# jhidalgocarrio/slam-localization

Hardware: AMD Instinct MI355X
Metric: filter predict+update steps/sec (higher is better)
Workload: dtype f64

## Files before the change

### slam-localization_amd/csrc/slk_kernels.hpp

```cpp
#pragma once
#include <hip/hip_runtime.h>

#include "../../include/slk.h"
#include "slk_math.hpp"

namespace slk {

typedef double d4 __attribute__((ext_vector_type(4)));
typedef float f4 __attribute__((ext_vector_type(4)));
typedef __bf16 b8 __attribute__((ext_vector_type(8)));

constexpr int KP = 8;
constexpr int STEP_WGS = 4;
constexpr int MAXM = 32;
constexpr int PRED_SCRATCH = 1536;

struct Lay { int kind, k, nfk, nfkl, N, Nq, nso3; };

struct KArgs {
    int B;
    Lay lay;
    double *mean; double *P; int *status; unsigned *outliers;
    int do_predict, pm; const double *u; int u_stride; const double *Q; int q_stride; const double *Yext;
    int do_update, mm; const double *mp; int mp_stride; const double *z; int m;
// ... 478 lines not shown
                        if (rho < kap) f = 0.0;
                        frag[I] = f;
                        if (rho >= kap && rho < n && kap < n) Lp[pk(n, rho, kap)] = f;
                    }
#pragma unroll
                    for (int J = JK; J < NT; ++J)
#pragma unroll
                        for (int I = J; I < NT; ++I)
                            acc[tile_idx(I, J)] = __builtin_amdgcn_mfma_f64_16x16x4f64(frag[I], frag[J], acc[tile_idx(I, J)], 0, 0, 0);
                }
            }
            CholMCols<NT, JK + 1>::run(acc, Lp, n, colbuf, lane, fail);
        }
    }
};

template <int NT>
__device__ __forceinline__ int cholm_factor(d4 (&acc)[CholM<NT>::NTL], double *Lp, int n, double *colbuf, int lane)
{
    int fail = -1;
    __builtin_amdgcn_s_setprio(3);
    CholMCols<NT, 0>::run(acc, Lp, n, colbuf, lane, fail);
    wave_sync();
    __builtin_amdgcn_s_setprio(0);
    return fail;
}

__device__ __forceinline__ double readlane_f64(double x, int l)
{
    return __hiloint2double(__builtin_amdgcn_readlane(__double2hiint(x), l), __builtin_amdgcn_readlane(__double2loint(x), l));
}

template <int J> __device__ __forceinline__ double row_bcast_const_f64(double x)
{
    return __builtin_amdgcn_update_dpp(0.0, x, 0x150 + J, 0xf, 0xf, true);
}
__device__ __forceinline__ double row_bcast_f64(double x, int j)
{
    switch (j & 15) {
    case 0: return row_bcast_const_f64<0>(x);
    case 1: return row_bcast_const_f64<1>(x);
    case 2: return row_bcast_const_f64<2>(x);
    case 3: return row_bcast_const_f64<3>(x);
    case 4: return row_bcast_const_f64<4>(x);
    case 5: return row_bcast_const_f64<5>(x);
    case 6: return row_bcast_const_f64<6>(x);
    case 7: return row_bcast_const_f64<7>(x);
    case 8: return row_bcast_const_f64<8>(x);
    case 9: return row_bcast_const_f64<9>(x);
    case 10: return row_bcast_const_f64<10>(x);
    case 11: return row_bcast_const_f64<11>(x);
    case 12: return row_bcast_const_f64<12>(x);
    case 13: return row_bcast_const_f64<13>(x);
    case 14: return row_bcast_const_f64<14>(x);
    default: return row_bcast_const_f64<15>(x);
    }
}

template <int LO, int HI, int OFF>
__device__ __forceinline__ void lds_store4_lane_ranges(unsigned addr, const double (&v)[4])
{
    constexpr int W0 = HI - LO > 0 ? HI - LO : 0, W1 = HI - LO - 1 > 0 ? HI - LO - 1 : 0;
    constexpr int W2 = HI - LO - 2 > 0 ? HI - LO - 2 : 0, W3 = HI - LO - 3 > 0 ? HI - LO - 3 : 0;
    static_assert(LO >= 0 && HI <= 64 && W0 < 64 && LO + 3 < 64 && OFF >= 0 && OFF + 384 < 65536, "s_bfm_b64 fields, ds offset");
    unsigned long long save;
    asm volatile("s_mov_b64 %[sv], exec\n\t"
                 "s_bfm_b64 exec, %[w0], %[l0]\n\tds_write_b64 %[a], %[v0] offset:%[o0]\n\t"
                 "s_bfm_b64 exec, %[w1], %[l1]\n\tds_write_b64 %[a], %[v1] offset:%[o1]\n\t"
                 "s_bfm_b64 exec, %[w2], %[l2]\n\tds_write_b64 %[a], %[v2] offset:%[o2]\n\t"
                 "s_bfm_b64 exec, %[w3], %[l3]\n\tds_write_b64 %[a], %[v3] offset:%[o3]\n\t"
                 "s_mov_b64 exec, %[sv]"
                 : [sv] "=&s"(save)
                 : [a] "v"(addr), [v0] "v"(v[0]), [v1] "v"(v[1]), [v2] "v"(v[2]), [v3] "v"(v[3]),
                   [w0] "n"(W0), [w1] "n"(W1), [w2] "n"(W2), [w3] "n"(W3), [l0] "n"(LO), [l1] "n"(LO + 1), [l2] "n"(LO + 2), [l3] "n"(LO + 3),
                   [o0] "n"(OFF), [o1] "n"(OFF + 128), [o2] "n"(OFF + 256), [o3] "n"(OFF + 384)
                 : "memory");
}

struct CholNoRelease { __device__ __forceinline__ void operator()() const { } };
template <int NT, int JK, int C0, int OUT = 1, int NC = 0>
struct CholPSteps {
    template <class RelFn>
    __device__ __forceinline__ static void run(d4 (&acc)[CholM<NT>::NTL], double *Lp, int n, double *colbuf, int lane, unsigned &bad,
                                               int ksync, RelFn &rel)
    {
        static_assert(OUT != 2 || (NC > 0 && NC <= 16 * NT), "the tile variant takes n as a template argument too");
        if constexpr (JK < NT) {
            constexpr int LDC = CholM<NT>::LDC;
            constexpr int k0 = 16 * JK + C0;
            if constexpr (OUT == 2) n = NC;
            if (k0 < n) {
                const int c = lane & 15, g = lane >> 4;
                const int row = (NT == 4) ? lane : min(lane, 16 * NT - 1);
                auto live = [&](int p) { return OUT != 2 || k0 + p < n; };
                const bool last = OUT == 2 && k0 + 4 >= n;
#pragma unroll
                for (int I = JK; I < NT; ++I) colbuf[g * LDC + 16 * I + c] = acc[tile_idx(I, JK)][C0 / 4];
                wave_sync();
                double m[4], l[4];
#pragma unroll
                for (int p = 0; p < 4; ++p) m[p] = live(p) ? colbuf[p * LDC + row] : 0.0;
#pragma unroll
                for (int p = 0; p < 4; ++p) {
                    l[p] = 0.0;
                    if (!live(p)) continue;
                    const double mpiv = readlane_f64(m[p], k0 + p), d = -mpiv;
                    {
                        if constexpr (OUT == 2) {
                            const unsigned rk = pivot_rank_neg((unsigned)__double2hiint(mpiv), (unsigned)__double2loint(mpiv));
                            bad = rk > bad ? rk : bad;
                            asm volatile("" : "+s"(bad));
                        } else {
                            int nb = !(d > 0.0);
                            asm volatile("" : "+v"(nb));
                            bad |= (nb != 0) ? 0x7ff00000u : 0u;
                        }
                    }
                    double sq, rs;
                    rsqrt_pivot(d, sq, rs);
                    (void)sq;
                    l[p] = m[p] * -rs;
#pragma unroll
                    for (int q = p + 1; q < 4; ++q)
                        if (live(q)) m[q] = fma(l[p], readlane_f64(l[p], k0 + q), m[q]);
                }
                if constexpr (OUT != 2) {
                    wave_sync();
                    if (NT == 4 || lane < 16 * NT) {
#pragma unroll
                        for (int p = 0; p < 4; ++p) colbuf[p * LDC + lane] = l[p];
                    }
                }
                if constexpr (OUT == 2) {
                    typedef __attribute__((address_space(3))) double ldouble;
                    const int It = lane >> 4;
                    const unsigned trow = (unsigned)(size_t)(ldouble *)Lp + (It * (It + 1) / 2 * 256 + (lane & 15)) * 8;
                    lds_store4_lane_ranges<k0, NC, (JK * 256 + C0 * 16) * 8>(trow, l);
                    if (ksync == k0 / 4) rel();
                }
#pragma unroll
                for (int p = 0; p < 4; ++p) {
                    if constexpr (OUT == 1) {
                        typedef __attribute__((address_space(1))) double gdouble;
                        unsigned long long colb = reinterpret_cast<unsigned long long>(Lp + pkcol(n, k0 + p));
                        asm volatile("" : "+s"(colb));
                        gdouble *colp = reinterpret_cast<gdouble *>(colb);
                        if (k0 + p < n && lane >= k0 + p && lane < n) colp[lane] = l[p];
                    } else if constexpr (OUT == 0) {
                        if (k0 + p < n && lane >= k0 + p && lane < n) Lp[pkcol(n, k0 + p) + lane] = l[p];
                    }
                }
                if (!last) {
                    constexpr int J0 = (C0 == 12) ? JK + 1 : JK;
                    wave_sync();
                    double frag[NT];
                    if constexpr (OUT == 2) {
#pragma unroll
                        for (int I = J0; I < NT; ++I) frag[I] = Lp[tile_idx(I, JK) * 256 + (C0 + g) * 16 + c];
                    } else {
#pragma unroll
                        for (int I = J0; I < NT; ++I) frag[I] = colbuf[g * LDC + 16 * I + c];
                        wave_sync();
                    }
#pragma unroll
                    for (int J = J0; J < NT; ++J)
#pragma unroll
                        for (int I = J; I < NT; ++I)
                            acc[tile_idx(I, J)] = __builtin_amdgcn_mfma_f64_16x16x4f64(frag[J], frag[I], acc[tile_idx(I, J)], 0, 0, 0);
                }
            }
            CholPSteps<NT, (C0 == 12 ? JK + 1 : JK), (C0 + 4) & 15, OUT, NC>::run(acc, Lp, n, colbuf, lane, bad, ksync, rel);
        }
    }
};

template <int NT, int OUT = 1, int NC = 0, class RelFn = CholNoRelease>
__device__ __forceinline__ int cholp_factor(d4 (&acc)[CholM<NT>::NTL], double *Lp, int n, double *colbuf, int lane, int ksync = -1,
                                            RelFn rel = RelFn())
{
    static_assert(OUT == 2 || std::is_same<RelFn, CholNoRelease>::value, "only the tile variant releases columns early");
    unsigned bad = 0u;
    CholPSteps<NT, 0, 0, OUT, NC>::run(acc, Lp, n, colbuf, lane, bad, ksync, rel);
    wave_sync();
    return pivot_rank_not_positive(bad) ? 0 : -1;
}

template <int NMAX, bool ROWB = false, class InitFn>
__device__ __forceinline__ int chol_rows(double *Lp, int n, int lane, InitFn init, int nst = -1)
{
    if (nst < 0) nst = n;
    static_assert(NMAX <= 32, "chol_rows keeps a row per lane in registers");
    static_assert(!ROWB || NMAX <= 16, "one matrix per DPP row of sixteen lanes");
    double a[NMAX];
#pragma unroll
    for (int j = 0; j < NMAX; ++j) {
        a[j] = init(min(lane, n - 1), j < n ? j : 0);
        if ((j & 3) == 3) __builtin_amdgcn_sched_barrier(0);
    }
    bool bad = false;
#pragma unroll
    for (int j = 0; j < NMAX; ++j) {
        if (j < n) {
            const double d = ROWB ? row_bcast_f64(a[j], j) : readlane_f64(a[j], j);
            bad |= !(d > 0.0);
            double sq, rs;
            rsqrt_pivot(d, sq, rs);
            (void)sq;
            a[j] *= rs;
#pragma unroll
            for (int k = j + 1; k < NMAX; ++k) a[k] = fma(-a[j], ROWB ? row_bcast_f64(a[j], k) : readlane_f64(a[j], k), a[k]);
            __builtin_amdgcn_sched_barrier(0);
        }
    }
    if (lane < nst) {
#pragma unroll
        for (int j = 0; j < NMAX; ++j)
            if (j < nst && lane >= j) Lp[pk(nst, lane, j)] = a[j];
    }
    wave_sync();
    return bad ? 0 : -1;
}

template <int NT, class InitFn>
__device__ __forceinline__ void cholw_load(d4 (&acc)[NT], int n, int lane, int wave, InitFn init)
{
    const int c = lane & 15, g = lane >> 4;
#pragma unroll
    for (int J = 0; J < NT; ++J)
#pragma unroll
        for (int r = 0; r < 4; ++r) {
            int row = 16 * wave + g + 4 * r, col = 16 * J + c;
            double v = 0.0;
            if (J <= wave && wave < NT) {
                if (row < n && col < n) v = (row >= col) ? init(row, col) : init(col, row);
                else v = (row == col) ? 1.0 : 0.0;
            }
            acc[J][r] = -v;
        }
}

template <int NT, class XFn, class YFn>
__device__ __forceinline__ void cholw_downdate(d4 (&acc)[NT], int n, int kk, int lane, int wave, XFn xel, YFn yel)
{
    const int c = lane & 15, g = lane >> 4;
    if (wave >= NT) return;
    for (int ks = 0; ks * 4 < kk; ++ks) {
        const int cc = 4 * ks + g;
        double bf[NT];
        const int rw = 16 * wave + c;
        const bool okw = cc < kk && rw < n;
        const double af = okw ? xel(rw, cc) : 0.0;
#pragma unroll
        for (int J = 0; J < NT; ++J) {
            int rho = 16 * J + c;
            bool ok = cc < kk && rho < n && J <= wave;
            bf[J] = ok ? yel(rho, cc) : 0.0;
        }
#pragma unroll
        for (int J = 0; J < NT; ++J)
            if (J <= wave) acc[J] = __builtin_amdgcn_mfma_f64_16x16x4f64(af, bf[J], acc[J], 0, 0, 0);
    }
}

template <int NT>
__device__ __forceinline__ int cholw_factor(d4 (&acc)[NT], double *Lp, int n, double *colbuf, double *coef, int lane,
// ... 2512 lines not shown
```

### slam-localization_amd/csrc/slk_math.hpp

```cpp
#pragma once
#include <hip/hip_runtime.h>

namespace slk {

struct Quat { double x, y, z, w; };

__device__ __forceinline__ Quat qmul(const Quat &a, const Quat &b)
{
    Quat o;
    o.w = a.w * b.w - a.x * b.x - a.y * b.y - a.z * b.z;
    o.x = a.w * b.x + a.x * b.w + a.y * b.z - a.z * b.y;
    o.y = a.w * b.y + a.y * b.w + a.z * b.x - a.x * b.z;
    o.z = a.w * b.z + a.z * b.w + a.x * b.y - a.y * b.x;
    return o;
}

__device__ __forceinline__ Quat qconj(const Quat &q) { return Quat{-q.x, -q.y, -q.z, q.w}; }

__device__ __forceinline__ void qrot(const Quat &q, double vx, double vy, double vz,
                                     double &ox, double &oy, double &oz)
{
    double ux = q.y * vz - q.z * vy, uy = q.z * vx - q.x * vz, uz = q.x * vy - q.y * vx;
    ux += ux; uy += uy; uz += uz;
    ox = vx + q.w * ux + (q.y * uz - q.z * uy);
    oy = vy + q.w * uy + (q.z * ux - q.x * uz);
    oz = vz + q.w * uz + (q.x * uy - q.y * ux);
}

__host__ __device__ __forceinline__ unsigned pivot_rank_neg(unsigned xhi, unsigned xlo)
{
#if defined(__HIP_DEVICE_COMPILE__)
    unsigned rk;
    asm("s_cmp_lg_u32 %2, 0\n\ts_addc_u32 %0, %1, 0x7fffffff" : "=s"(rk) : "s"(xhi), "s"(xlo) : "scc");
    return rk;
#else
    return xhi + 0x7fffffffu + (xlo != 0u ? 1u : 0u);
#endif
}
__host__ __device__ __forceinline__ bool pivot_rank_not_positive(unsigned rank) { return rank >= 0x7ff00000u; }
__host__ __device__ __forceinline__ bool pivot_not_positive(unsigned hi, unsigned lo) { return pivot_rank_not_positive(pivot_rank_neg(hi ^ 0x80000000u, lo)); }

constexpr double MEAN_STOP_SQ = 0x1.19799812dea11p-40;

__host__ __device__ __forceinline__ bool nonneg_hi_below(unsigned xhi, unsigned bound_hi) { return xhi < bound_hi; }
constexpr unsigned HI_QUARTER = 0x3fd00000u, HI_FOUR = 0x40100000u;

struct CosSinc { double c, s; };
__device__ __forceinline__ CosSinc cos_sinc_sqrt_libm_body(double x)
{
    const double sx = sqrt(x);
    return CosSinc{cos(sx), sin(sx) / sx};
}
__device__ __forceinline__ double so3_log_scale_libm_body(double n2, double w)
{
    double nv = sqrt(n2);
    if (nv < 1e-11) nv = 1e-11;
    return 2.0 / nv * atan(nv / w);
}
__device__ __attribute__((noinline)) CosSinc cos_sinc_sqrt_libm(double x) { return cos_sinc_sqrt_libm_body(x); }
__device__ __attribute__((noinline)) double so3_log_scale_libm(double n2, double w) { return so3_log_scale_libm_body(n2, w); }

template <bool LEAF = false>
__device__ __forceinline__ void cos_sinc_sqrt(double x, double &c, double &s)
{
    if (x < 0.25) {
        const double y = -x;
        double cc = 0x1.1d8d32755f8fbp-29;
        cc = fma(cc, y, 0x1.27e40964b47d4p-22);
        cc = fma(cc, y, 0x1.a01a00fb1bc6fp-16);
        cc = fma(cc, y, 0x1.6c16c16bdd04ep-10);
        cc = fma(cc, y, 0x1.5555555555421p-5);
        cc = fma(cc, y, 0x1.fffffffffffffp-2);
        cc = fma(cc, y, 1.0);
        double ss = 0x1.ac53ce336f805p-26;
        ss = fma(ss, y, 0x1.71dd113fb7905p-19);
        ss = fma(ss, y, 0x1.a01a01061c190p-13);
        ss = fma(ss, y, 0x1.11111110ecfb3p-7);
        ss = fma(ss, y, 0x1.555555555548fp-3);
        ss = fma(ss, y, 1.0);
        c = cc;
        s = ss;
    } else {
        const CosSinc r = LEAF ? cos_sinc_sqrt_libm_body(x) : cos_sinc_sqrt_libm(x);
        c = r.c;
        s = r.s;
    }
}

template <bool LEAF = false>
__device__ __forceinline__ Quat so3_exp(double vx, double vy, double vz)
{
    double c, s;
    cos_sinc_sqrt<LEAF>(0.25 * (vx * vx + vy * vy + vz * vz), c, s);
    double m = s * 0.5;
    return Quat{m * vx, m * vy, m * vz, c};
}

__device__ __forceinline__ double rcp_refined(double a)
{
    const double r0 = __builtin_amdgcn_rcp(a);
    const double e = fma(-a, r0, 1.0);
    return fma(fma(e, e, e), r0, r0);
}

template <bool LEAF = false>
__device__ __forceinline__ void so3_log(const Quat &q, double &vx, double &vy, double &vz)
{
    const double n2 = q.x * q.x + q.y * q.y + q.z * q.z;
    const double w2 = q.w * q.w;
    double s;
    if (q.w > 0.0 && n2 * 16.0 < w2) {
        const double rw = rcp_refined(q.w);
        const double y = -(n2 * rw * rw);
        double f = 0x1.78be0a9b1dd1fp-5;
        f = fma(f, y, 0x1.0b3340fe2ed9ap-4);
        f = fma(f, y, 0x1.3ab708d770276p-4);
        f = fma(f, y, 0x1.7459b99bfc19bp-4);
        f = fma(f, y, 0x1.c71c5f4b9c2adp-4);
        f = fma(f, y, 0x1.24924907fa636p-3);
        f = fma(f, y, 0x1.999999996d307p-3);
        f = fma(f, y, 0x1.5555555555481p-2);
        f = fma(f, y, 1.0);
        s = 2.0 * f * rw;
    } else {
        s = LEAF ? so3_log_scale_libm_body(n2, q.w) : so3_log_scale_libm(n2, q.w);
// ... 92 lines not shown
```

### slam-localization_amd/csrc/slk_step_fast.hpp

```cpp
#pragma once
#ifdef SLK_STAMPS
#define SLK_FSTAMP(i) do { SLK_STAMP_NR(i); if (a.stop > 0 && a.stop == (i)) return true; } while (0)
#define SLK_WSTAMP(w, i) do { if (tid == 64 * (w) && a.dbg) a.dbg[(size_t)bidx * 32 + (i)] = clock64(); } while (0)
#define SLK_FBAIL(code) do { SLK_NOTE(28, code); return false; } while (0)
#else
#define SLK_FSTAMP(i) do { } while (0)
#define SLK_WSTAMP(w, i) do { } while (0)
#define SLK_FBAIL(code) return false
#endif

namespace slk {

template <int I> struct FastIdx { static constexpr int value = I; };
template <int B, int E, class F> __device__ __forceinline__ void fast_steps_to(int last, F &&f)
{
    if constexpr (B < E) {
        if (B <= last) {
            f(FastIdx<B>());
            fast_steps_to<B + 1, E>(last, f);
        }
    }
}

template <int K> struct FastShape {
    static constexpr int N = 12 + 6 * K, Nq = 13 + 7 * K, S = 2 * N + 1, NSO3 = K + 1;
    static constexpr int NT = (N + 15) / 16, NTL = NT * (NT + 1) / 2, NKS = (N + 3) / 4;
    static constexpr int NROT = 3 * NSO3;
    static constexpr int NP = 3 * K * K + 15 * K + 6;
    static constexpr int NIT = NP + NSO3;
    static constexpr int RND = (NIT + 255) / 256;
    static constexpr int oLt = 0;
    static constexpr int oMu = oLt + NTL * 256;
    static constexpr int oRef = oMu + ((Nq + 7) & ~7);
    static constexpr int oDelta = oRef + ((Nq + 7) & ~7);
    static constexpr int oMd = oDelta + 64;
    static constexpr int oD0 = oMd + 32;
    static constexpr int oD0s = oD0 + 32;
    static constexpr int oPd = oD0s + 32;
    static constexpr int oCq = oPd + 64;
    static constexpr int oStr = oCq + 40;
    static constexpr int oInts = oStr + 64;
    static constexpr int oTab = oInts + 32;
    static constexpr int oMsq = oTab + 28;
    static constexpr int oU = oTab + 32;
    static constexpr int uYp = 0, uW = 0, uDZ = 1088, uSm = 1600, uMdiag = 1664, uB = 1728, uInnov = 1792, uDz0 = 1800, uTmp = 1808;
    static constexpr int USZ = (NKS * 128 > 1936) ? NKS * 128 : 1936;
    static constexpr int total = oU + USZ;
};

static_assert(FastShape<8>::total * 8 * 4 <= 160 * 1024 && FastShape<7>::total * 8 * 4 <= 160 * 1024, "four workgroups per CU");

__host__ __device__ inline int fast_step_lds_doubles(int k)
{
    switch (k) {
    case 4: return FastShape<4>::total;
    case 5: return FastShape<5>::total;
    case 6: return FastShape<6>::total;
    case 7: return FastShape<7>::total;
    case 8: return FastShape<8>::total;
    default: return 0;
    }
}

__device__ __forceinline__ double wave_sum_f64(double x) { return readlane_f64(wave_inclusive_scan(x), 63); }

template <int N> __device__ __forceinline__ int fast_rho(int t)
{
    if (t >= N) return 31;
    if (t < 12) return (t >= 3 && t < 6) ? t - 3 : 31;
    const int cc = (t - 12) / 6, r = (t - 12) - 6 * cc;
    return r >= 3 ? 3 * cc + r : 31;
}
__device__ __forceinline__ int fast_vec_storage(int t)
{
    if (t < 12) return t < 3 ? t : (t < 6 ? -1 : t + 1);
    const int cc = (t - 12) / 6, r = (t - 12) - 6 * cc;
    return r < 3 ? 13 + 7 * cc + r : -1;
}

__device__ const double fast_series_table[26] = {
    0x1.1d8d32755f8fbp-29, 0x1.27e40964b47d4p-22, 0x1.a01a00fb1bc6fp-16, 0x1.6c16c16bdd04ep-10, 0x1.5555555555421p-5, 0x1.fffffffffffffp-2,
    0x1.ac53ce336f805p-26, 0x1.71dd113fb7905p-19, 0x1.a01a01061c190p-13, 0x1.11111110ecfb3p-7, 0x1.555555555548fp-3,
    0x1.78be0a9b1dd1fp-5, 0x1.0b3340fe2ed9ap-4, 0x1.3ab708d770276p-4, 0x1.7459b99bfc19bp-4, 0x1.c71c5f4b9c2adp-4, 0x1.24924907fa636p-3, 0x1.999999996d307p-3, 0x1.5555555555481p-2,
    0.0, 0.0, 0.0, 0.0, 0.0, 0.0, 0.0};

__device__ __forceinline__ bool wave_all(bool p) { return __builtin_amdgcn_ballot_w64(!p) == 0ull; }

template <int NV, bool WIDE>
__device__ __forceinline__ void so3_exp_tab_path(const double *T, const double (&v)[NV][3], const double (&x)[NV], Quat (&q)[NV])
{
    double y[NV], cc[NV], ss[NV];
// ... 431 lines not shown
__device__ __forceinline__ void fast_rebuild_col(const double *Lt, const double *str, int lane, d4 (&acc)[FastShape<K>::NT])
{
    using F = FastShape<K>;
    constexpr int NT = F::NT;
    constexpr int KEND = (4 * J + 4 + (J == 0 ? 1 : 0) < F::NKS) ? 4 * J + 4 + (J == 0 ? 1 : 0) : F::NKS;
#pragma unroll
    for (int ks = 0; ks < KEND; ++ks) {
        double fo[NT];
#pragma unroll
        for (int I = J; I < NT; ++I) {
            const int Kc = ks >> 2;
            fo[I] = (Kc <= I) ? Lt[(I * (I + 1) / 2 + Kc) * 256 + (ks & 3) * 64 + lane] : str[lane];
        }
#pragma unroll
        for (int I = J; I < NT; ++I) acc[I - J] = __builtin_amdgcn_mfma_f64_16x16x4f64(fo[I], fo[J], acc[I - J], 0, 0, 0);
    }
}

template <int K, int J>
__device__ __forceinline__ void fast_store_col(const double *ee, double *bufs, double *oP, int lane, d4 (&acc)[FastShape<K>::NT],
                                               bool lower_only)
{
    using F = FastShape<K>;
    constexpr int NT = F::NT, N = F::N, EES = FastEE<K>::EES, PAD = FastEE<K>::PAD;
    const int c = lane & 15, g = lane >> 4;
    {
        const int rj = fast_rho<N>(16 * J + c);
        const double *eec = ee + (rj & PAD);
#pragma unroll
        for (int I = J; I < NT; ++I) {
            const unsigned rw = g == 0 ? fast_rho_pack<K>(I, 0) : (g == 1 ? fast_rho_pack<K>(I, 1) : (g == 2 ? fast_rho_pack<K>(I, 2) : fast_rho_pack<K>(I, 3)));
#pragma unroll
            for (int r = 0; r < 4; ++r) acc[I - J][r] += eec[((rw >> (8 * r)) & 0xffu) * EES];
        }
    }
    double *o = oP + c + g * N;
#pragma unroll
    for (int I = J; I < NT; ++I) {
#pragma unroll
        for (int r = 0; r < 4; ++r) {
            const bool full = 16 * I + 4 * r + 3 < N && 16 * J + 15 < N;
            if (I > J && lower_only) continue;
            if (16 * I + 4 * r < N && (full || (16 * I + 4 * r + g < N && 16 * J + c < N)))
                o[16 * J + (16 * I + 4 * r) * N] = acc[I - J][r];
        }
        if (I > J) {
            double *buf = bufs + (I * (I - 1) / 2 + J) * 272;
#pragma unroll
            for (int r = 0; r < 4; ++r) buf[c * 17 + g + 4 * r] = acc[I - J][r];
            wave_sync();
#pragma unroll
            for (int q = 0; q < 4; ++q) {
                const double v = buf[(g + 4 * q) * 17 + c];
                const bool full = 16 * I + 15 < N;
                if (full || 16 * I + c < N) o[16 * I + (16 * J + 4 * q) * N] = v;
            }
        }
    }
}

template <int K>
__device__ __forceinline__ bool msckf_step_fast(const KArgs &a, double *smem)
{
    using F = FastShape<K>;
    constexpr int N = F::N, Nq = F::Nq, S = F::S, NSO3 = F::NSO3, NT = F::NT, NKS = F::NKS, NROT = F::NROT;
    constexpr int NP = F::NP;
    constexpr int NTHREADS = 256;
    if (a.mm != SLK_MM_FEATURE_PROJ || a.gate == 2 || a.emit != 0 || a.rebuild_prec != 0 || !a.mp || a.m != 8) return false;
    const int bidx = blockIdx.x, tid = threadIdx.x, lane = tid & 63;
    const int wave = __builtin_amdgcn_readfirstlane(tid >> 6);
    const int c16 = lane & 15, g4 = lane >> 4;
    double *Lt = smem + F::oLt, *mu = smem + F::oMu, *ref = smem + F::oRef, *delta = smem + F::oDelta, *md32 = smem + F::oMd;
    double *d0 = smem + F::oD0, *d0s = smem + F::oD0s, *pd = smem + F::oPd, *cq = smem + F::oCq, *str = smem + F::oStr, *U = smem + F::oU;
    int *ints = reinterpret_cast<int *>(smem + F::oInts);
    double *T = smem + F::oTab, *msq = smem + F::oMsq;
    double *Yp = U + F::uYp, *Wb = U + F::uW, *dZi = U + F::uDZ, *Sm = U + F::uSm, *mdiag = U + F::uMdiag, *bvec = U + F::uB;
    double *innov = U + F::uInnov, *dz0 = U + F::uDz0, *tmpS = U + F::uTmp, *Et = U;
    const double *gmean = a.mean + (size_t)bidx * Nq;
    const double *gP = a.P + (size_t)bidx * N * N;
    const double *mp = a.mp + (size_t)bidx * a.mp_stride;
    SLK_STAMP_NR(0);

    int jmax = 0, ksmax, bad;
    const bool here = a.wsfail == nullptr;
    {
        const double *gL = here ? gP : a.wsL + (size_t)bidx * pk_size(N);
        const int t = lane, It = t >> 4;
        const int lbase = (It * (It + 1) / 2) * 256 + wave * 16 + (t & 15);
        double v[16];
        if (!here) {
#pragma unroll
            for (int u = 0; u < 16; ++u) {
                const int j = 4 * u + wave;
                const bool in = j < N && t >= j && t < N;
                v[u] = gL[in ? pkcol(N, j) + t : 0];
            }
        }
        const double mu0 = (tid < Nq) ? gmean[tid] : 0.0;
        const int t0 = (tid && tid < NSO3) ? 9 + 6 * tid : 3;
        const double pdg = gP[t0 * (N + 1)] + gP[(t0 + 1) * (N + 1)] + gP[(t0 + 2) * (N + 1)];
        const double tabv = fast_series_table[tid < 26 ? tid : 25];
        bad = here ? 0 : (a.wsfail[bidx] >= 0);
        bool ok = true;
#pragma unroll
        for (int f = 0; f < 4; ++f) {
            const double cf = mp[4 * f + 3];
            ok = ok && (cf >= 0.0) && (cf <= (double)K);
            const int cp = ok ? (int)cf : 0, tp = cp ? 6 + 6 * cp : 0;
            jmax = (tp + 5 > jmax) ? tp + 5 : jmax;
        }
        jmax = __builtin_amdgcn_readfirstlane(jmax);
        ksmax = jmax >> 2;
        bad |= !ok;
        if (tid < NSO3) bad |= !(pdg < 9.869604401089358);
        if (tid < Nq) mu[tid] = mu0;
        if (tid < 64) ints[tid] = 0;
        if (tid < 26) T[tid] = tabv;
        if (!here) {
#pragma unroll
            for (int u = 0; u < 16; ++u) {
                const int j = 4 * u + wave;
                const bool in = j < N && t >= j && t < N;
                if ((u >> 2) < NT && It >= (u >> 2) && It < NT) Lt[lbase + (u >> 2) * 256 + (u & 3) * 64] = in ? v[u] : 0.0;
            }
        }
        if (here) {
            d4 fa[CholM<NT>::NTL];
            if (wave == 0) cholm_load_t_exact<NT, N>(fa, gP, lane);
            else {
                double2 *Lt2 = reinterpret_cast<double2 *>(Lt);
                for (int e = tid - 64; e < CholM<NT>::NTL * 128; e += NTHREADS - 64) Lt2[e] = double2{0.0, 0.0};
            }
            __syncthreads();
            static_assert(CholM<NT>::COLBUF <= F::oStr + 64 - F::oRef, "colbuf fits the arrays of the gain phase and the mean loop");
            if (wave == 0) {
                bad |= cholp_factor<NT, 2, N>(fa, Lt, N, ref, lane, ksmax, [&]() __attribute__((always_inline)) {
                    wave_sync();
                    __builtin_amdgcn_s_barrier();
                    SLK_WSTAMP(0, 16);
                }) >= 0;
            } else {
                __syncthreads();
            }
        } else {
            __syncthreads();
        }
    }
    SLK_FSTAMP(3);

    const bool second = ksmax + 3 < NKS;
    int f = wave;
    for (bool go = wave != 0 || !second; go; go = second && f == 1, f = 0) {
        if (f == wave) { SLK_WSTAMP(0, 17); SLK_WSTAMP(1, 19); }
        const double cf = mp[4 * f + 3];
        const int cp = (cf >= 0.0 && cf <= (double)K) ? (int)cf : 0;
        const int tp = cp ? 6 + 6 * cp : 0, sp = cp ? 6 + 7 * cp : 0;
        const double fx = mp[4 * f], fy = mp[4 * f + 1], fz = mp[4 * f + 2];
        const int j = lane, Jc = j >> 4;
        const bool act = j < tp + 6;
        double l[6], x[7];
#pragma unroll
        for (int q = 0; q < 6; ++q) {
            const int t = tp + q, I = t >> 4;
            const bool in = act && Jc <= I;
            l[q] = Lt[in ? (I * (I + 1) / 2 + Jc) * 256 + (j & 15) * 16 + (t & 15) : 16];
        }
#pragma unroll
        for (int q = 0; q < 7; ++q) x[q] = mu[sp + q];
        double zp0, zp1, zm0, zm1;
        {
            const double rv[2][3] = {{l[3], l[4], l[5]}, {-l[3], -l[4], -l[5]}};
            Quat ex[2];
            so3_exp_tab_flag<2>(T, rv, ex, ints + 50);
            const Quat qx = Quat{x[3], x[4], x[5], x[6]};
            double lx, ly, lz;
            auto quot = [](double lx_, double ly_, double lz_, double &q0, double &q1) __attribute__((always_inline)) {
                const double r = rcp_refined(lz_);
                q0 = lx_ * r; q0 = fma(fma(-lz_, q0, lx_), r, q0);
                q1 = ly_ * r; q1 = fma(fma(-lz_, q1, ly_), r, q1);
            };
            qrot(qconj(qmul_exp(qx, ex[0])), fx - (x[0] + l[0]), fy - (x[1] + l[1]), fz - (x[2] + l[2]), lx, ly, lz);
            quot(lx, ly, lz, zp0, zp1);
            qrot(qconj(qmul_exp(qx, ex[1])), fx - (x[0] - l[0]), fy - (x[1] - l[1]), fz - (x[2] - l[2]), lx, ly, lz);
            quot(lx, ly, lz, zm0, zm1);
        }
        const double Z00 = readlane_f64(zp0, 63), Z01 = readlane_f64(zp1, 63);
        const double yp0 = zp0 - Z00, yp1 = zp1 - Z01, ym0 = zm0 - Z00, ym1 = zm1 - Z01;
        Yp[j * 17 + 2 * f] = yp0; Yp[j * 17 + 2 * f + 1] = yp1;
        Yp[j * 17 + 8 + 2 * f] = ym0; Yp[j * 17 + 8 + 2 * f + 1] = ym1;
        dZi[f * 128 + 2 * j] = yp0 - ym0; dZi[f * 128 + 2 * j + 1] = yp1 - ym1;
        const double s0 = wave_sum_f64(yp0 + ym0), s1 = wave_sum_f64(yp1 + ym1);
        if (lane == 0) {
            const double e0 = s0 * (1.0 / (double)S), e1 = s1 * (1.0 / (double)S);
            innov[2 * f] = a.z[(size_t)bidx * 8 + 2 * f] - (Z00 + e0);
            innov[2 * f + 1] = a.z[(size_t)bidx * 8 + 2 * f + 1] - (Z01 + e1);
            dz0[2 * f] = e0; dz0[2 * f + 1] = e1;
        }
        SLK_WSTAMP(0, 18); SLK_WSTAMP(1, 21);
    }
    if (__syncthreads_or(bad)) SLK_FBAIL(2);
    if (ints[50]) SLK_FBAIL(3);
    if (tid < 64) { str[tid] = 0.0; pd[tid] = 0.0; }
    if (tid < 32) { d0[tid] = 0.0; md32[tid] = 0.0; }
    SLK_FSTAMP(4);

    double Gs[NKS - 1], Gt[36];
    if (wave == 1) {
        d4 acc = {0.0, 0.0, 0.0, 0.0};
        fast_steps_to<0, NKS>(ksmax, [&](auto ix) __attribute__((always_inline)) {
            constexpr int ks = decltype(ix)::value;
            const double fr = Yp[ks * 68 + g4 * 17 + c16];
            acc = __builtin_amdgcn_mfma_f64_16x16x4f64(fr, fr, acc, 0, 0, 0);
        });
        if (c16 < 8) { tmpS[g4 + 8 * c16] = acc[0]; tmpS[g4 + 4 + 8 * c16] = acc[1]; }
        else { tmpS[64 + g4 + 8 * (c16 - 8)] = acc[2]; tmpS[64 + g4 + 4 + 8 * (c16 - 8)] = acc[3]; }
        wave_sync();
        const double *R = a.R + (size_t)bidx * a.r_stride;
        const int row = lane & 7, col = lane >> 3;
        Sm[lane] = 0.5 * ((tmpS[lane] + tmpS[64 + lane]) - (double)S * dz0[row] * dz0[col]) + R[lane];
    } else if (wave == 3) {
        fast_prefix_tail(dZi, lane, Gt);
        __builtin_amdgcn_sched_barrier(0);
        fast_prefix_blocks<NKS>(dZi, c16, g4, Gs);
    }
    __syncthreads();
    SLK_FSTAMP(6);
    if (wave == 3) {
        fast_prefix_park<NKS>(Yp, c16, g4, ksmax, Gs);
        wave_sync();
    }

    unsigned kept = 0xffu, nout = 0u;
    if (a.gate) {
        const int p = 2 * (lane & 3), q = p + 1;
        const double s00 = Sm[p + 8 * p], s01 = Sm[p + 8 * q], s10 = Sm[q + 8 * p], s11 = Sm[q + 8 * q];
        const double det = s00 * s11 - s01 * s10, r0 = innov[p], r1 = innov[q];
        const double d2 = (r0 * (s11 * r0 - s01 * r1) + r1 * (s00 * r1 - s10 * r0)) / det;
        if (!__all(d2 < 5.99)) {
            int *ix = ints + 10 * wave;
            if (lane == 0) {
                int cnt = 8, i = 0;
                unsigned no = 0;
                for (int r = 0; r < 8; ++r) ix[r] = r;
                while (i < cnt / 2) {
                    const int pp = ix[2 * i], qq = ix[2 * i + 1];
                    const double t00 = Sm[pp + 8 * pp], t01 = Sm[pp + 8 * qq], t10 = Sm[qq + 8 * pp], t11 = Sm[qq + 8 * qq];
                    const double dt = t00 * t11 - t01 * t10, u0 = innov[pp], u1 = innov[qq];
                    const double dd = (u0 * (t11 * u0 - t01 * u1) + u1 * (t00 * u1 - t10 * u0)) / dt;
                    if (!(dd < 5.99)) {
                        for (int rep = 0; rep < 2; ++rep) {
                            const int pos = 2 * i + rep, numRows = cnt - 1;
                            if (pos < numRows) for (int w = pos; w < numRows; ++w) ix[w] = ix[w + 1];
                            cnt = numRows;
                        }
                        no++;
                    } else {
                        i++;
                    }
                }
                unsigned kp = 0;
                for (int r = 0; r < cnt; ++r) kp |= 1u << ix[r];
                ix[8] = (int)kp; ix[9] = (int)no;
            }
            wave_sync();
            kept = (unsigned)ix[8]; nout = (unsigned)ix[9];
        }
    }
    if (kept == 0u) SLK_FBAIL(4);
    SLK_FSTAMP(7);

    if (wave == 0) {
        double gg[8][8], gi[8], y[8];
        if (kept == 0xffu) {
#pragma unroll
            for (int i = 0; i < 8; ++i) {
#pragma unroll
                for (int j = 0; j <= i; ++j) gg[i][j] = Sm[i + 8 * j];
            }
        } else {
#pragma unroll
            for (int i = 0; i < 8; ++i) {
#pragma unroll
                for (int j = 0; j <= i; ++j) {
                    const bool in = ((kept >> i) & 1u) && ((kept >> j) & 1u);
                    const double v = Sm[in ? i + 8 * j : 0];
                    gg[i][j] = in ? v : (i == j ? 1.0 : 0.0);
                }
            }
        }
        bool spd = true;
#pragma unroll
        for (int j = 0; j < 8; ++j) {
            double d = gg[j][j];
#pragma unroll
            for (int p = 0; p < j; ++p) d = fma(-gg[j][p], gg[j][p], d);
            spd = spd && (d > 0.0);
            double sq, rs;
            rsqrt_pivot(d, sq, rs);
            gi[j] = rs;
#pragma unroll
            for (int i = j + 1; i < 8; ++i) {
                double v = gg[i][j];
#pragma unroll
                for (int p = 0; p < j; ++p) v = fma(-gg[i][p], gg[j][p], v);
                gg[i][j] = v * rs;
            }
            double s = ((kept >> j) & 1u) ? innov[j] : 0.0;
#pragma unroll
// ... 274 lines not shown
```

Before: 26.77 million.

## Stagger feature projections across waves via early Cholesky column release plan

Replaces the single Cholesky release point with a bitmask of release steps computed from the per-feature column indices. Waves can start projecting the features whose Cholesky columns are already final while wave 0 continues factoring, and the innovation-covariance build can run before the phase-1 barrier. This is meant to overlap the measurement sigma-point work with the Cholesky tail and remove a barrier round. In exchange it adds plan computation and extra barrier-matching paths, which raises the risk of barrier-count mismatches between waves.

```diff
diff --git a/slam-localization_amd/csrc/slk_kernels.hpp b/slam-localization_amd/csrc/slk_kernels.hpp
--- a/slam-localization_amd/csrc/slk_kernels.hpp
+++ b/slam-localization_amd/csrc/slk_kernels.hpp
@@ -584,7 +584,7 @@
 struct CholPSteps {
     template <class RelFn>
     __device__ __forceinline__ static void run(d4 (&acc)[CholM<NT>::NTL], double *Lp, int n, double *colbuf, int lane, unsigned &bad,
-                                               int ksync, RelFn &rel)
+                                               unsigned relmask, RelFn &rel)
     {
         static_assert(OUT != 2 || (NC > 0 && NC <= 16 * NT), "the tile variant takes n as a template argument too");
         if constexpr (JK < NT) {
@@ -638,7 +638,7 @@
                     const int It = lane >> 4;
                     const unsigned trow = (unsigned)(size_t)(ldouble *)Lp + (It * (It + 1) / 2 * 256 + (lane & 15)) * 8;
                     lds_store4_lane_ranges<k0, NC, (JK * 256 + C0 * 16) * 8>(trow, l);
-                    if (ksync == k0 / 4) rel();
+                    if (relmask & (1u << (k0 / 4))) rel();
                 }
 #pragma unroll
                 for (int p = 0; p < 4; ++p) {
@@ -671,18 +671,18 @@
                             acc[tile_idx(I, J)] = __builtin_amdgcn_mfma_f64_16x16x4f64(frag[J], frag[I], acc[tile_idx(I, J)], 0, 0, 0);
                 }
             }
-            CholPSteps<NT, (C0 == 12 ? JK + 1 : JK), (C0 + 4) & 15, OUT, NC>::run(acc, Lp, n, colbuf, lane, bad, ksync, rel);
+            CholPSteps<NT, (C0 == 12 ? JK + 1 : JK), (C0 + 4) & 15, OUT, NC>::run(acc, Lp, n, colbuf, lane, bad, relmask, rel);
         }
     }
 };
 
 template <int NT, int OUT = 1, int NC = 0, class RelFn = CholNoRelease>
-__device__ __forceinline__ int cholp_factor(d4 (&acc)[CholM<NT>::NTL], double *Lp, int n, double *colbuf, int lane, int ksync = -1,
+__device__ __forceinline__ int cholp_factor(d4 (&acc)[CholM<NT>::NTL], double *Lp, int n, double *colbuf, int lane, unsigned relmask = 0u,
                                             RelFn rel = RelFn())
 {
     static_assert(OUT == 2 || std::is_same<RelFn, CholNoRelease>::value, "only the tile variant releases columns early");
     unsigned bad = 0u;
-    CholPSteps<NT, 0, 0, OUT, NC>::run(acc, Lp, n, colbuf, lane, bad, ksync, rel);
+    CholPSteps<NT, 0, 0, OUT, NC>::run(acc, Lp, n, colbuf, lane, bad, relmask, rel);
     wave_sync();
     return pivot_rank_not_positive(bad) ? 0 : -1;
 }
diff --git a/slam-localization_amd/csrc/slk_math.hpp b/slam-localization_amd/csrc/slk_math.hpp
--- a/slam-localization_amd/csrc/slk_math.hpp
+++ b/slam-localization_amd/csrc/slk_math.hpp
@@ -41,6 +41,41 @@
 __host__ __device__ __forceinline__ bool pivot_not_positive(unsigned hi, unsigned lo) { return pivot_rank_not_positive(pivot_rank_neg(hi ^ 0x80000000u, lo)); }
 
 constexpr double MEAN_STOP_SQ = 0x1.19799812dea11p-40;
+
+struct FastReleasePlan {
+    unsigned mask;
+    unsigned word;
+};
+constexpr int FAST_HX_STEPS = 3, FAST_PLAN_NONE = 7;
+__host__ __device__ __forceinline__ FastReleasePlan fast_release_plan(int c0, int c1, int c2, int c3, int K, int hc, bool need_c)
+{
+    const int nks = (12 + 6 * K + 3) >> 2;
+    auto key = [](int c, int f) { return ((((c ? 6 + 6 * c : 0) + 5) >> 2) << 2) | f; };
+    int k0 = key(c0, 0), k1 = key(c1, 1), k2 = key(c2, 2), k3 = key(c3, 3);
+    auto cx = [](int &a, int &b) { const int lo = a < b ? a : b, hi = a < b ? b : a; a = lo; b = hi; };
+    cx(k0, k1); cx(k2, k3); cx(k0, k2); cx(k1, k3); cx(k1, k2);
+    const int ra = k1 >> 2, ksmax = k3 >> 2;
+    const unsigned none = (unsigned)FAST_PLAN_NONE;
+    auto pack = [](unsigned w0p0, unsigned w0p1, unsigned w1p0, unsigned w1p1, unsigned w2p0, unsigned w2p1, unsigned w3p0, unsigned w3p1) {
+        return w0p0 | (w0p1 << 3) | (w1p0 << 6) | (w1p1 << 9) | (w2p0 << 12) | (w2p1 << 15) | (w3p0 << 18) | (w3p1 << 21);
+    };
+    FastReleasePlan p;
+    const int c = ksmax + hc;
+    const bool hasc = hc > 0 && c <= nks - 2;
+    if (ra + FAST_HX_STEPS <= ksmax && (hasc || !need_c)) {
+        p.mask = (1u << ra) | (1u << ksmax) | (hasc ? 1u << c : 0u);
+        p.word = pack(none, none, (unsigned)k0 & 3u, (unsigned)k2 & 3u, (unsigned)k1 & 3u, (unsigned)k3 & 3u, none, none) | (1u << 24) |
+                 (hasc ? 1u << 25 : 0u);
+    } else {
+        const bool second = ksmax + FAST_HX_STEPS < nks;
+        p.mask = 1u << ksmax;
+        p.word = pack(second ? none : 0u, none, 1u, second ? 0u : none, 2u, none, 3u, none);
+    }
+    return p;
+}
+__host__ __device__ __forceinline__ int fast_plan_feature(const FastReleasePlan &p, int wave, int pass) { return (int)((p.word >> (6 * wave + 3 * pass)) & 7u); }
+__host__ __device__ __forceinline__ bool fast_plan_staggered(const FastReleasePlan &p) { return (p.word >> 24) & 1u; }
+__host__ __device__ __forceinline__ bool fast_plan_has_c(const FastReleasePlan &p) { return (p.word >> 25) & 1u; }
 
 __host__ __device__ __forceinline__ bool nonneg_hi_below(unsigned xhi, unsigned bound_hi) { return xhi < bound_hi; }
 constexpr unsigned HI_QUARTER = 0x3fd00000u, HI_FOUR = 0x40100000u;
diff --git a/slam-localization_amd/csrc/slk_step_fast.hpp b/slam-localization_amd/csrc/slk_step_fast.hpp
--- a/slam-localization_amd/csrc/slk_step_fast.hpp
+++ b/slam-localization_amd/csrc/slk_step_fast.hpp
@@ -7,6 +7,13 @@
 #define SLK_FSTAMP(i) do { } while (0)
 #define SLK_WSTAMP(w, i) do { } while (0)
 #define SLK_FBAIL(code) return false
+#endif
+
+#ifndef SLK_RELEASE_HC
+#define SLK_RELEASE_HC 3
+#endif
+#ifndef SLK_RELEASE_NEED_C
+#define SLK_RELEASE_NEED_C 1
 #endif
 
 namespace slk {
@@ -604,6 +611,7 @@
     SLK_STAMP_NR(0);
 
     int jmax = 0, ksmax, bad;
+    FastReleasePlan plan;
     const bool here = a.wsfail == nullptr;
     {
         const double *gL = here ? gP : a.wsL + (size_t)bidx * pk_size(N);
@@ -624,15 +632,25 @@
         const double tabv = fast_series_table[tid < 26 ? tid : 25];
         bad = here ? 0 : (a.wsfail[bidx] >= 0);
         bool ok = true;
+        int cps[4], cmax = 0;
 #pragma unroll
         for (int f = 0; f < 4; ++f) {
             const double cf = mp[4 * f + 3];
-            ok = ok && (cf >= 0.0) && (cf <= (double)K);
-            const int cp = ok ? (int)cf : 0, tp = cp ? 6 + 6 * cp : 0;
-            jmax = (tp + 5 > jmax) ? tp + 5 : jmax;
-        }
-        jmax = __builtin_amdgcn_readfirstlane(jmax);
+            const bool in = (cf >= 0.0) && (cf <= (double)K);
+            ok = ok && in;
+            cps[f] = __builtin_amdgcn_readfirstlane(in ? (int)cf : 0);
+            cmax = cps[f] > cmax ? cps[f] : cmax;
+        }
+        jmax = __builtin_amdgcn_readfirstlane((cmax ? 6 + 6 * cmax : 0) + 5);
         ksmax = jmax >> 2;
+        bool single = !here;
+#ifdef SLK_STAMPS
+        single = single || a.stop == 3;
+#endif
+        plan = single ? fast_release_plan(cmax, cmax, cmax, cmax, K, 0, true)
+                      : fast_release_plan(cps[0], cps[1], cps[2], cps[3], K, SLK_RELEASE_HC, SLK_RELEASE_NEED_C != 0);
+        plan.mask = (unsigned)__builtin_amdgcn_readfirstlane((int)plan.mask);
+        plan.word = (unsigned)__builtin_amdgcn_readfirstlane((int)plan.word);
         bad |= !ok;
         if (tid < NSO3) bad |= !(pdg < 9.869604401089358);
         if (tid < Nq) mu[tid] = mu0;
@@ -656,10 +674,19 @@
             __syncthreads();
             static_assert(CholM<NT>::COLBUF <= F::oStr + 64 - F::oRef, "colbuf fits the arrays of the gain phase and the mean loop");
             if (wave == 0) {
-                bad |= cholp_factor<NT, 2, N>(fa, Lt, N, ref, lane, ksmax, [&]() __attribute__((always_inline)) {
+#ifdef SLK_STAMPS
+                int nrel = 0;
+#endif
+                bad |= cholp_factor<NT, 2, N>(fa, Lt, N, ref, lane, plan.mask, [&]() __attribute__((always_inline)) {
                     wave_sync();
+#ifdef SLK_STAMPS
+                    SLK_WSTAMP(0, nrel == 0 ? 1 : (nrel == 1 ? 9 : 5));
+#endif
                     __builtin_amdgcn_s_barrier();
-                    SLK_WSTAMP(0, 16);
+#ifdef SLK_STAMPS
+                    SLK_WSTAMP(0, nrel == 0 ? 2 : (nrel == 1 ? 10 : 31));
+                    ++nrel;
+#endif
                 }) >= 0;
             } else {
                 __syncthreads();
@@ -670,10 +697,13 @@
     }
     SLK_FSTAMP(3);
 
-    const bool second = ksmax + 3 < NKS;
-    int f = wave;
-    for (bool go = wave != 0 || !second; go; go = second && f == 1, f = 0) {
-        if (f == wave) { SLK_WSTAMP(0, 17); SLK_WSTAMP(1, 19); }
+    const bool staggered = fast_plan_staggered(plan);
+#pragma nounroll
+    for (int pass = 0; pass < 2; ++pass) {
+        if (pass == 1 && staggered && wave != 0) __syncthreads();
+        const int f = fast_plan_feature(plan, wave, pass);
+        if (f == FAST_PLAN_NONE) continue;
+        if (pass == 0) { SLK_WSTAMP(0, 17); SLK_WSTAMP(1, 19); }
         const double cf = mp[4 * f + 3];
         const int cp = (cf >= 0.0 && cf <= (double)K) ? (int)cf : 0;
         const int tp = cp ? 6 + 6 * cp : 0, sp = cp ? 6 + 7 * cp : 0;
@@ -720,13 +750,21 @@
         }
         SLK_WSTAMP(0, 18); SLK_WSTAMP(1, 21);
     }
-    if (__syncthreads_or(bad)) SLK_FBAIL(2);
-    if (ints[50]) SLK_FBAIL(3);
-    if (tid < 64) { str[tid] = 0.0; pd[tid] = 0.0; }
-    if (tid < 32) { d0[tid] = 0.0; md32[tid] = 0.0; }
-    SLK_FSTAMP(4);
-
     double Gs[NKS - 1], Gt[36];
+    const bool early_s = fast_plan_has_c(plan);
+    auto close_phase1 = [&]() __attribute__((always_inline)) {
+        if (__syncthreads_or(bad)) return 2;
+        if (ints[50]) return 3;
+        if (tid < 64) { str[tid] = 0.0; pd[tid] = 0.0; }
+        if (tid < 32) { d0[tid] = 0.0; md32[tid] = 0.0; }
+        return 0;
+    };
+    if (!early_s) {
+        if (const int code = close_phase1()) SLK_FBAIL(code);
+        SLK_FSTAMP(4);
+    } else if (wave != 0) {
+        __syncthreads();
+    }
     if (wave == 1) {
         d4 acc = {0.0, 0.0, 0.0, 0.0};
         fast_steps_to<0, NKS>(ksmax, [&](auto ix) __attribute__((always_inline)) {
@@ -740,12 +778,18 @@
         const double *R = a.R + (size_t)bidx * a.r_stride;
         const int row = lane & 7, col = lane >> 3;
         Sm[lane] = 0.5 * ((tmpS[lane] + tmpS[64 + lane]) - (double)S * dz0[row] * dz0[col]) + R[lane];
+        SLK_WSTAMP(1, 16);
     } else if (wave == 3) {
         fast_prefix_tail(dZi, lane, Gt);
         __builtin_amdgcn_sched_barrier(0);
         fast_prefix_blocks<NKS>(dZi, c16, g4, Gs);
     }
-    __syncthreads();
+    if (early_s) {
+        if (const int code = close_phase1()) SLK_FBAIL(code);
+        SLK_FSTAMP(4);
+    } else {
+        __syncthreads();
+    }
     SLK_FSTAMP(6);
     if (wave == 3) {
         fast_prefix_park<NKS>(Yp, c16, g4, ksmax, Gs);
```

Measured after the change: 27.23 million, median of 6. +1.7%, better.
